# fabriziosestito/policy-server

Measured on AMD Instinct MI355X. Metric: admission requests evaluated/sec (node) at 64 policies; HBM GB/s vs peak, higher is better.
Workload: dtype u8; 1 GPU; C4: 1000000 synthetic Pod AdmissionReviews per GPU x 64 compiled policies (c4_64.yml: 22 psp-capabilities, 21 psp-apparmor, 21 safe-labels); config=c4_64, total_requests=1000000, policies=64, parallelism=dp1 (request shards)

## Files before the change

include/kwgpu.h:

```cpp
#ifndef KWGPU_H
#define KWGPU_H

#include <stddef.h>
#include <stdint.h>

#ifdef __cplusplus
extern "C" {
#endif

enum {
  KW_OK = 0,
  KW_E_INVALID_ID = 1,
  KW_E_INIT = 2,
  KW_E_NOT_FOUND = 3,
  KW_E_BOOTSTRAP = 4,
  KW_E_ENGINE = 5,
  KW_E_GROUP_REHYDRATE = 6,
  KW_E_ARG = 16,
  KW_E_PAYLOAD = 17,
  KW_E_DEVICE = 18,
  KW_E_NOSPACE = 19
};

enum { KW_MODE_PROTECT = 0, KW_MODE_MONITOR = 1 };
// ... 124 lines not shown
                       int origin, uint32_t *out);

int kw_debug_plan(const kw_env *env, kw_batch *b, const int32_t *policies, uint32_t npol, int origin, uint32_t *out,
                  int cap);

int kw_debug_copy_jobs(const kw_env *env, kw_batch *b, const int32_t *policies, uint32_t npol, int origin,
                       uint32_t *out, size_t cap, size_t *needed);

int kw_debug_tile_descs(const kw_env *env, kw_batch *b, const int32_t *policies, uint32_t npol, int origin,
                        uint32_t *out, size_t cap, size_t *needed);

uint64_t kw_debug_tile_cost(uint32_t feat, uint32_t need, uint32_t requests, uint32_t labels, uint32_t containers,
                            uint32_t capabilities);

int kw_debug_tile_slot(uint64_t ndesc, uint32_t grid, uint32_t workgroup, uint32_t tile, uint64_t *out);

int kw_debug_reorder(const kw_batch *b, uint64_t *perm, size_t cap, uint64_t *split, kw_batch **out);

int kw_validate_batch(const kw_env *env, kw_batch *b, const int32_t *policies, uint32_t npol,
                      int origin, void *stream);
int kw_validate_rows(const kw_env *env, kw_batch *b, const int32_t *row_policy, int origin,
                     void *stream);
int kw_batch_verdicts(kw_batch *b, uint32_t *host_out, size_t count);
int kw_validate_host(const kw_env *env, kw_batch *b, const int32_t *policies, uint32_t npol, int origin,
                     int device, uint32_t *out, size_t count, uint32_t chunk_rows);
typedef struct kw_packed {
  uint64_t rows;
  uint32_t npol;
  uint64_t *planes;
  uint32_t *exc_off;
// ... 83 lines not shown
```

policy-server_amd/csrc/capi.cpp:

```cpp
#include <hip/hip_runtime.h>

#include <algorithm>
#include <cstdio>
#include <cstdlib>
#include <cstring>
#include <memory>
#include <string>
#include <thread>
#include <vector>

#include "../../include/kwgpu.h"
#include "automaton.hpp"
#include "batch.hpp"
#include "devbatch.hpp"
#include "env.hpp"
#include "kernels.hpp"
#include "knobs.hpp"
#include "metrics.hpp"
#include "pass.hpp"
#include "plan.hpp"
#include "service.hpp"
#include "slotplan.hpp"
#include "upload.hpp"
#include "yaml.hpp"
// ... 633 lines not shown
}

uint64_t kw_debug_tile_cost(uint32_t feat, uint32_t need, uint32_t requests, uint32_t labels, uint32_t containers,
                            uint32_t capabilities) {
  return tile_cost(tile_cost_weights(feat, need), requests, labels, containers, capabilities);
}

int kw_debug_tile_slot(uint64_t ndesc, uint32_t grid, uint32_t workgroup, uint32_t tile, uint64_t* out) {
  if (!out || !grid || workgroup >= grid) return KW_E_ARG;
  const TileSlot s = tile_slot(ndesc, grid, workgroup);
  const uint64_t v[7] = {s.nx, s.xcd, s.slot, s.wpx, s.t_lo, s.t_hi, tile_at(s, tile)};
  std::copy(v, v + 7, out);
  return KW_OK;
}

int kw_debug_reorder(const kw_batch* kb, uint64_t* perm, size_t cap, uint64_t* split, kw_batch** out) {
  if (!kb || !split || !out || (!perm && kb->b.n) || cap < kb->b.n) return KW_E_ARG;
  std::vector<uint64_t> p;
  *split = split_rows(kb->b, &p);
  if (!*split) {
    p.resize(kb->b.n);
    for (uint64_t r = 0; r < kb->b.n; ++r) p[r] = r;
  }
  auto nb = std::make_unique<kw_batch>();
  RowOrder o;
  permute_batch(kb->b, p, &nb->b, true, &o);
  std::copy(p.begin(), p.end(), perm);
  *out = nb.release();
  return KW_OK;
}
// ... 136 lines not shown
```

policy-server_amd/csrc/devbatch.hpp:

```cpp
#pragma once
#include <hip/hip_runtime.h>

#include <atomic>
#include <cstdint>
#include <deque>
#include <memory>
#include <utility>
#include <vector>

#include "../../include/kwgpu.h"
#include "batch.hpp"
#include "env.hpp"
#include "kernels.hpp"
#include "pools.hpp"
#include "slotplan.hpp"

struct kw_env {
  kw::Env e;
  uint64_t uid = next_uid();
  static uint64_t next_uid() {
    static std::atomic<uint64_t> n{1};
    return n++;
  }
};
// ... 76 lines not shown
  uint32_t* verdicts = nullptr;
  size_t verdict_cap = 0;
  size_t last_verdicts = 0;
  uint32_t last_row_words = 0;
  std::vector<uint64_t> perm;
  std::vector<uint64_t> inv_perm;
  uint64_t split = 0;
  std::unique_ptr<Batch> dev_b;
  std::shared_ptr<PassPlan> plan_cache;
  uint64_t plan_env = 0, plan_knobs = 0;
  std::vector<int32_t> plan_pols;
  int plan_origin = -1;
  std::unique_ptr<RowOrder> order;
  uint32_t loaded = 0;
  uint32_t* sched = nullptr;
  hipEvent_t ev[3] = {nullptr, nullptr, nullptr};
  TileArgs* d_tiles = nullptr;
  size_t d_tiles_cap = 0;
  std::vector<TileArgs> h_tiles;
  uint8_t* d_slots = nullptr;
  size_t d_slots_cap = 0;
  std::vector<uint8_t> h_slots;
  uint32_t* rowcol = nullptr;
  size_t rowcol_cap = 0;
  std::vector<uint32_t> h_rowcol;
  TileDesc* desc = nullptr;
  size_t desc_cap = 0;
  uint32_t* overflow = nullptr;
  size_t overflow_cap = 0;
  std::vector<TileDesc> h_desc;
// ... 105 lines not shown
```

policy-server_amd/csrc/kernels.hip:

```cpp
#include <hip/hip_runtime.h>

#include <algorithm>
#include <array>
#include <cstddef>
#include <mutex>

#include "../../include/kwgpu.h"
#include "imgscan.hpp"
#include "kernels.hpp"


namespace kw {

typedef uint32_t u32x4 __attribute__((ext_vector_type(4)));

__device__ inline uint32_t lit_word(const uint32_t* base, uint32_t i, uint32_t sh, uint32_t len) {
  const uint32_t w = align_bytes(base[i + 1], base[i], sh);
  const uint32_t rem = len - 4u * i;
  return rem >= 4u ? w : (w & ((1u << (8u * rem)) - 1u));
}

template <bool BATCH, int N = 8>
__device__ inline uint32_t lit_lookup(const uint8_t* rec, const uint8_t* bytes, uint32_t b, uint32_t e) {
  const DevLit* L = (const DevLit*)rec;
// ... 433 lines not shown
  uint32_t* l_nx = (uint32_t*)(lds + t.o_nx);
  TileDesc* l_desc = (TileDesc*)(lds + t.o_desc);
  auto fetch_desc = [&](uint64_t i, uint32_t s) {
    if (tid < 32u)
      __builtin_amdgcn_global_load_lds((const __attribute__((address_space(1))) void*)((const uint32_t*)(desc + i) + tid),
                                       (__attribute__((address_space(3))) void*)(l_desc + s), 4, 0, 0);
  };
  auto sfield = [](const uint32_t& f) -> uint32_t { return __builtin_amdgcn_readfirstlane(f); };
  constexpr bool DYNB = !IMG;
  auto next_block = [&](uint32_t k) -> uint32_t {
    uint32_t v = 0;
    if (lane == 0u) v = atomicAdd(&l_nx[2u + k], 1u);
    return (kSlotThreads >> 6) + __builtin_amdgcn_readfirstlane(v);
  };
  const uint32_t wpx = (gridDim.x - xcd + nx - 1u) / nx;
  const uint64_t dbase = t_lo + 2ull * wpx;
  uint64_t tile = t_lo + blockIdx.x / nx, next = tile + wpx;
  constexpr bool desc_early = LDST;
  if (desc_early && tile < t_hi) fetch_desc(tile, 0);
  if (LDST) {
    for (uint32_t s = 0; s < t.nstage; ++s)
      glds_x4((const u32x4*)(a.blob + t.stage_blob[s]), (u32x4*)(lds + t.stage_lds[s]), t.stage_bytes[s] / 16u, tid);
    for (uint32_t c = 0; c < t.nchunk; ++c)
      glds_x4((const u32x4*)t.chunk[c].rec, (u32x4*)(lds + t.chunk[c].o_lds), ((const SlotHdr*)t.chunk[c].rec)->staged / 16u, tid);
  }
  __syncthreads();
  mark(7);
  const uint8_t* tb = LDST ? (const uint8_t*)lds : a.blob;
  Classifiers C;
#pragma unroll
  for (int c = 0; c < (int)NCOL; ++c) {
// ... 53 lines not shown
    const CopyJob q = tp->jobs[lane];
    jb_lo = (uint32_t)q.base;
    jb_hi = (uint32_t)(q.base >> 32);
    jb_code = q.code;
  }

  if (!desc_early) {
    if (tile < t_hi) fetch_desc(tile, 0);
    __syncthreads();
  }
  mark(4);
  for (uint32_t it = 0; tile < t_hi; ++it) {
    const uint64_t p0_t0 = timing ? clock64() : 0;
    const uint32_t cur = it & 1u;
    uint32_t nxt2 = 0;
    if (dyn && tid == 0) nxt2 = atomicAdd(cnt, 1u);
    if (next < t_hi) fetch_desc(next, cur ^ 1u);
    const TileDesc& d = l_desc[cur];
#define KW_DF(x) sfield(x)
    if (!KW_DF(d.fits)) {
      if (dyn && tid == 0) l_nx[cur] = nxt2;
      __syncthreads();
      tile = next;
      next = dyn ? dbase + l_nx[cur] : next + wpx;
      continue;
    }
    uint64_t p0_t1 = 0, p0_t2 = 0;
    if (timing) {
      p0_t1 = clock64();
      sg_add(SG_P0_TOP, p0_t1 - p0_t0);
    }

    {
      const uint32_t* dw = (const uint32_t*)&d;
      uint32_t code_v = jb_code;
      asm volatile("" : "+v"(code_v));
      const CopySpan sp = copy_span(code_v, dw[code_v & 31u], dw[(code_v >> 5) & 31u], d.r0hi);
      const uint64_t src = (((uint64_t)jb_hi << 32) | jb_lo) + sp.byte_off;
      const uint32_t s_lo = (uint32_t)src, s_hi = (uint32_t)(src >> 32);
// ... 563 lines not shown
          }
        }
      }
      if (timing) sg_add(SG_P3_BUSY, clock64() - p3_t0);
      if (ck + 1 < t.nchunk) {
        if (DYNB && tid == 0) l_nx[3] = 0;
        lds_barrier();
        mark(4);
      }
    }
    const uint64_t p3_end = timing ? clock64() : 0;
    lds_barrier();
    if (timing) sg_add(SG_P3_WAIT, clock64() - p3_end);
    mark(4);
    tile = next;
    next = dyn ? dbase + l_nx[cur] : next + wpx;
  }
  if (timing && tid == 0) {
    ph[6] = clock64() - t_begin;
    a.phase[(uint64_t)blockIdx.x * kPhaseWords + 8u + SG_END] = __builtin_amdgcn_s_memrealtime();
    for (int k = 0; k < 8; ++k) a.phase[(uint64_t)blockIdx.x * kPhaseWords + (uint32_t)k] = ph[k];
  }
  if (dyn && tid == 0) {
    uint32_t* done = a.sched + 256u + xcd * 32u;
    __threadfence();
    if (atomicAdd(done, 1u) == wpx - 1u) {
      atomicExch(cnt, 0u);
      atomicExch(done, 0u);
    }
  }
  (void)lane;
  (void)wave;
}

constexpr int kOverflowThreads = 256;

__device__ inline Classifiers blob_classifiers(const EvalArgs& a, const TileArgs& t) {
  Classifiers C;
  for (int c = 0; c < (int)NCOL; ++c) {
    C.lit[c] = t.lit_blob[c] ? a.blob + t.lit_blob[c] : nullptr;
// ... 322 lines not shown
  if (dev < 0 || dev >= kMaxDevices) return hipErrorInvalidDevice;
  std::call_once(g_attr_once[dev], [dev] {
    hipError_t e = hipSuccess;
    for (int k = 0; k < 70; ++k) {
      const uint32_t feat = k < 64 ? (uint32_t)(k >> 2) & kFeatAll : k < 68 ? (kFeatAll | kFeatNfa) : (kFeatLbl | kFeatCtr | kFeatRng);
      const hipError_t ek =
          hipFuncSetAttribute(tile_fn(k & 1, (k & 2) != 0, feat), hipFuncAttributeMaxDynamicSharedMemorySize, 160 * 1024);
      if (e == hipSuccess) e = ek;
    }
    g_attr_err[dev] = e;
  });
  return g_attr_err[dev];
}
}

hipError_t launch_evaluate_tiles(const EvalArgs& a, const TileArgs& t, const TileArgs* d_t, const TileDesc* d_desc,
                                 uint32_t grid, hipStream_t s) {
  if (a.nrows == 0 || t.nchunk == 0 || a.ndesc == 0) return hipSuccess;
  if (hipError_t e = ensure_attrs(); e != hipSuccess) return e;
  {
    thread_local int c_dev = -1, c_ncu = 0, c_occ = 0;
    thread_local uint64_t c_key = ~0ull;
    int dev = 0;
    const uint64_t key = ((uint64_t)t.lds_bytes << 8) | ((uint64_t)tile_feat(t) << 2) | (a.phase ? 2u : 0u) | (t.lds_tables ? 1u : 0u);
    if (hipGetDevice(&dev) == hipSuccess && (dev != c_dev || key != c_key)) {
      int ncu = 0, occ = 0;
      const void* fn = tile_fn(t.lds_tables != 0, a.phase != nullptr, tile_feat(t));
      if (hipDeviceGetAttribute(&ncu, hipDeviceAttributeMultiprocessorCount, dev) != hipSuccess ||
          hipOccupancyMaxActiveBlocksPerMultiprocessor(&occ, fn, kSlotThreads, t.lds_bytes) != hipSuccess)
        ncu = occ = 0;
      c_dev = dev;
      c_key = key;
      c_ncu = ncu;
      c_occ = occ;
    }
    c_occ = std::min<int>(c_occ, (int)lds_workgroups_per_cu(t.lds_bytes));
    if (c_occ > 0 && c_ncu > 0) grid = std::max<uint32_t>(1u, std::min<uint32_t>(grid, (uint32_t)(c_occ * c_ncu)));
    if (t.debug & 256u)
      fprintf(stderr, "[kw tile] launch grid=%u occupancy=%d wg/cu x %d CUs lds=%u\n", grid, c_occ, c_ncu, t.lds_bytes);
  }
  using TileFn = void (*)(EvalArgs, const TileArgs*, const TileDesc*);
  const TileFn fn = (TileFn)tile_fn(t.lds_tables != 0, a.phase != nullptr, tile_feat(t));
  hipLaunchKernelGGL(fn, dim3(grid), dim3(kSlotThreads), t.lds_bytes, s, a, d_t, d_desc);
  return hipGetLastError();
}

__global__ void __launch_bounds__(256) scatter_kernel(ScatterArgs a) {
  const uint64_t tid = (uint64_t)blockIdx.x * 256u + threadIdx.x, nt = (uint64_t)gridDim.x * 256u;
  for (uint32_t k = 0; k < a.nseg; ++k) {
    const ScatterSeg g = a.seg[k];
    uint8_t* d = a.dst + g.dst_off;
    const uint8_t* s = a.src + g.src_off;
    const uint64_t head = std::min<uint64_t>(g.bytes, (16u - ((uintptr_t)d & 15u)) & 15u);
    const uint64_t words = (g.bytes - head) / 16u, tail = g.bytes - head - words * 16u;
    if (tid < head) d[tid] = s[tid];
// ... 327 lines not shown
```

policy-server_amd/csrc/kernels.hpp:

```cpp
#pragma once
#include <hip/hip_runtime.h>

#include <cstdint>

#include "kwdev.hpp"
#include "packed.hpp"
#include "slots.hpp"
#include "summary.hpp"

namespace kw {

enum Str : uint32_t { S_NS = 0, S_IMG, S_AA, S_CAPADD, S_CAPDROP, S_LK, S_LV, NSTR };

struct WideRec {
  uint32_t row_lo, row_hi, policy, value;
};

struct EvalArgs {
  const uint8_t* blob;
  uint64_t nrows;
  uint64_t ndesc;
  uint32_t npol;
  int32_t origin;
  const uint8_t* req_flags;
  const uint32_t* ctr_off;
  const uint32_t* lbl_off;
  const uint8_t* ctr_flags;
  const uint32_t* capadd_off;
  const uint32_t* capdrop_off;
  uint32_t* out;
  uint32_t* sched;
  uint16_t *g_ns, *g_aa, *g_img, *g_capadd, *g_capdrop, *g_lk, *g_lv;
  const uint16_t *nfa_lv, *nfa_img;
  uint32_t* wide_count;
  WideRec* wide_rec;
  uint32_t wide_cap;
  uint64_t* wide_groups;
  uint32_t nwide;
  const uint32_t* rowcol;
  uint64_t* phase;
};
enum Seg : uint32_t {
  SG_P1_LABEL = 0, SG_P1_CAPSTR, SG_P1_CTR, SG_P1_IMAGE, SG_P1_REQ, SG_P2_CTR, SG_P2_LABEL, SG_P2_REQ,
  SG_P1_BUSY, SG_P1_WAIT, SG_P2_BUSY, SG_P2_WAIT, SG_P0_WAIT, SG_P3_BUSY, SG_P3_WAIT,
  SG_START,
  SG_P0_TOP, SG_P0_REQ, SG_P0_STR,
// ... 110 lines not shown
struct TileSlot {
  uint32_t nx, xcd, slot, wpx;
  uint64_t t_lo, t_hi;
};
KW_HD inline TileSlot tile_slot(uint64_t ndesc, uint32_t grid, uint32_t b) {
  TileSlot s;
  s.nx = grid < 8u ? grid : 8u;
  s.xcd = b % s.nx;
  s.slot = b / s.nx;
  s.wpx = (grid - s.xcd + s.nx - 1u) / s.nx;
  s.t_lo = ndesc * s.xcd / s.nx;
  s.t_hi = ndesc * (s.xcd + 1u) / s.nx;
  return s;
}
KW_HD inline uint64_t tile_at(const TileSlot& s, uint32_t k) { return s.t_lo + s.slot + (uint64_t)k * s.wpx; }

struct TileCostW {
  uint32_t fixed, req, lbl, ctr, cap;
};
KW_HD constexpr uint32_t tile_blocks(uint32_t items) { return (items + 63u) / 64u; }
KW_HD constexpr uint64_t tile_cost(const TileCostW& w, uint32_t nreq, uint32_t nlbl, uint32_t nctr, uint32_t ncap) {
  return (uint64_t)w.fixed + (uint64_t)w.req * tile_blocks(nreq) + (uint64_t)w.lbl * tile_blocks(nlbl) +
         (uint64_t)w.ctr * tile_blocks(nctr) + (uint64_t)w.cap * tile_blocks(ncap);
}
KW_HD constexpr TileCostW tile_cost_weights(uint32_t feat, uint32_t need) {
  TileCostW w{47000u, 8450u, 0u, 0u, 0u};
  if ((feat & kFeatLbl) && (need & (1u << S_LK))) w.lbl = 9960u;
  if (feat & kFeatCtr) w.ctr = 10600u;
  if ((feat & kFeatCtr) && (need & (1u << S_CAPADD))) w.cap = 2750u;
  if ((feat & kFeatImg) && (need & (1u << S_IMG))) w.ctr = 35600u;
  return w;
}

void build_copy_jobs(TileArgs* T, const void* const cols[6]);

hipError_t launch_evaluate_tiles(const EvalArgs& a, const TileArgs& t, const TileArgs* d_t, const TileDesc* d_desc,
                                 uint32_t grid, hipStream_t s);
struct WideGroupArgs {
  uint32_t prog_off, prog_len;
  uint32_t col;
  uint32_t nmem, midx_off;
  uint32_t okw, rejb;
  uint32_t cause_off, cause_words;
  uint32_t errw;
  uint32_t kind;
  uint32_t mutw;
};

constexpr uint32_t kSplitMember = 0x80000000u;
// ... 97 lines not shown
```

policy-server_amd/csrc/knobs.hpp:

```cpp
#pragma once
#include <climits>
#include <cstddef>
#include <cstdint>

namespace kw {

enum Knob : int {
  KW_STREAM_POOL, KW_HOST_THREADS, KW_L2_PREFETCH, KW_KV_GLOBAL, KW_NO_MPACK,
  KW_BULK_DEBUG, KW_BULK_SAMPLE, KW_BULK_PACK, KW_BULK_CHUNK, KW_BULK_RAMP, KW_BULK_DIRECT, KW_BULK_DEPTH,
  KW_SCHED, KW_SPLIT, KW_GROUP_FORM, KW_POISON_VERDICTS, KW_FLATTEN_THREADS,
  KW_SLOT_ROWS, KW_HEAVY_ROWS, KW_HEAVY_CTR, KW_GLOBAL_TABLES, KW_TILE_SPLIT, KW_ROUND_SPLIT,
  KW_TILE_QUANTILE, KW_TILE_DEBUG, KW_TILE_CUT,
  KW_NKNOBS
};

enum class KnobKind : uint8_t {
  On,
  Off,
  Present,
  Int,
  Double,
  Str
};

struct KnobRow {
// ... 21 lines not shown

constexpr KnobRow kKnobs[KW_NKNOBS] = {
    knob_flag("KW_STREAM_POOL", KnobKind::On, kLatched, kNoPlan, "reuse streams and events per device"),
    knob_int("KW_HOST_THREADS", kLatched, kNoPlan, 0, 1, INT_MAX, kClamp, "host worker threads (unset: the hardware's, at most 16)"),
    knob_flag("KW_L2_PREFETCH", KnobKind::Off, kLatched, kPlans, "run the next-tile L2 prefetch (kernels built with KW_PREFETCH)"),
    knob_flag("KW_KV_GLOBAL", KnobKind::Off, kLatched, kPlans, "label-value DFAs read from global memory, not staged"),
    knob_flag("KW_NO_MPACK", KnobKind::Present, kLatched, kPlans, "slot plans without mandatory-field batching"),
    knob_flag("KW_BULK_DEBUG", KnobKind::Off, kLatched, kNoPlan, "print host stage times of planning and the bulk path"),
    knob_flag("KW_BULK_SAMPLE", KnobKind::On, kLatched, kNoPlan, "bulk path: tile capacities from ~2048 sampled tiles"),
    knob_flag("KW_BULK_PACK", KnobKind::On, kLatched, kNoPlan, "bulk path: packed chunks through their own ring"),
    knob_int("KW_BULK_CHUNK", kLatched, kNoPlan, 262144, 1, INT_MAX, kClamp, "bulk path: rows per chunk"),
    knob_flag("KW_BULK_RAMP", KnobKind::On, kLatched, kNoPlan, "bulk path: small first and last chunks"),
    knob_flag("KW_BULK_DIRECT", KnobKind::On, kLatched, kNoPlan, "bulk path: read back straight into pinned output"),
    knob_int("KW_BULK_DEPTH", kLatched, kNoPlan, -1, 0, INT_MAX, kClamp, "bulk path: chunks in flight (0: unbounded; unset: 2 or 3)"),
    knob_flag("KW_SCHED", KnobKind::Str, kLive, kPlans, "static / dynamic: force one tile schedule"),
    knob_int("KW_SPLIT", kLive, kPlans, -1, INT_MIN, INT_MAX, kClamp, "0: never split light / heavy rows, 1: whenever both exist"),
    knob_flag("KW_GROUP_FORM", KnobKind::Str, kLive, kPlans, "script: compile every group expression as a script"),
    knob_flag("KW_POISON_VERDICTS", KnobKind::Off, kLive, kPlans, "fill the verdict words with a sentinel before a pass"),
    knob_int("KW_FLATTEN_THREADS", kLive, kNoPlan, 0, 1, INT_MAX, kClamp, "JSON flatten threads (unset: the hardware's, at most 16)"),
    knob_int("KW_SLOT_ROWS", kLive, kPlans, 0, 8, 255, kElseUnset, "force the tile height"),
    knob_int("KW_HEAVY_ROWS", kLive, kPlans, 0, 8, 255, kElseUnset, "force the heavy region's tile height"),
    knob_int("KW_HEAVY_CTR", kLive, kPlans, 5, 1, INT_MAX, kElseUnset, "containers above which a request is heavy"),
    knob_flag("KW_GLOBAL_TABLES", KnobKind::Off, kLive, kPlans, "classifier tables read from global memory"),
    knob_real("KW_TILE_SPLIT", kPlans, 0.02, "share of tiles a capacity choice may split"),
    knob_real("KW_ROUND_SPLIT", kPlans, 0.02, "share of a taller tile's tiles that may need a second P1 round"),
    knob_real("KW_TILE_QUANTILE", kPlans, 0.0, "force the capacity quantile (unset: chosen per batch)"),
    knob_int("KW_TILE_DEBUG", kLive, kPlans, 0, INT_MIN, INT_MAX, kClamp, "kernel phase ablation bits; 256: print the plan"),
    knob_flag("KW_TILE_CUT", KnobKind::On, kLive, kPlans, "end each tile at the row of least estimated cost per row (0: fixed height)"),
};

constexpr bool knob_name_is(const char* a, const char* b) {
  while (*a && *a == *b) ++a, ++b;
  return *a == *b;
}
#define KW_KNOB_ROW(K) static_assert(knob_name_is(kKnobs[K].name, #K), "kKnobs is not in Knob order")
KW_KNOB_ROW(KW_STREAM_POOL); KW_KNOB_ROW(KW_HOST_THREADS); KW_KNOB_ROW(KW_L2_PREFETCH); KW_KNOB_ROW(KW_KV_GLOBAL);
KW_KNOB_ROW(KW_NO_MPACK); KW_KNOB_ROW(KW_BULK_DEBUG); KW_KNOB_ROW(KW_BULK_SAMPLE); KW_KNOB_ROW(KW_BULK_PACK);
KW_KNOB_ROW(KW_BULK_CHUNK); KW_KNOB_ROW(KW_BULK_RAMP); KW_KNOB_ROW(KW_BULK_DIRECT); KW_KNOB_ROW(KW_BULK_DEPTH);
KW_KNOB_ROW(KW_SCHED); KW_KNOB_ROW(KW_SPLIT); KW_KNOB_ROW(KW_GROUP_FORM); KW_KNOB_ROW(KW_POISON_VERDICTS);
KW_KNOB_ROW(KW_FLATTEN_THREADS); KW_KNOB_ROW(KW_SLOT_ROWS); KW_KNOB_ROW(KW_HEAVY_ROWS); KW_KNOB_ROW(KW_HEAVY_CTR);
KW_KNOB_ROW(KW_GLOBAL_TABLES); KW_KNOB_ROW(KW_TILE_SPLIT); KW_KNOB_ROW(KW_ROUND_SPLIT); KW_KNOB_ROW(KW_TILE_QUANTILE);
KW_KNOB_ROW(KW_TILE_DEBUG); KW_KNOB_ROW(KW_TILE_CUT);
#undef KW_KNOB_ROW

uint64_t kw_knob_hash();

namespace knob_detail {

const char* env(const KnobRow& r);
bool parse_bool(const KnobRow& r);
int parse_int(const KnobRow& r);
double parse_double(const KnobRow& r);

template <Knob K>
// ... 60 lines not shown
```

policy-server_amd/csrc/pass.cpp:

```cpp
#include "pass.hpp"

#include <atomic>
#include <chrono>
#include <cstdio>
#include <cstring>
#include <memory>

#include "knobs.hpp"
#include "plan.hpp"

namespace kw {

int upload_env(kw_env* env, int device) {
  if (device < 0) return KW_OK;
  HIPCHK(hipSetDevice(device));
  HIPCHK(hipMalloc(&env->e.d_blob, env->e.blob.size()));
  HIPCHK(hipMemcpy(env->e.d_blob, env->e.blob.data(), env->e.blob.size(), hipMemcpyHostToDevice));
  env->e.device = device;
  return KW_OK;
}

int build_descs(const Batch& B, const TileArgs& T, uint64_t lo, uint64_t hi, uint64_t t0, uint64_t t1, uint64_t range,
                uint32_t grid, std::vector<TileDesc>* desc, std::vector<uint32_t>* ovf) {
  auto make = [&](uint64_t r0, uint64_t r1, TileDesc* dp) {
// ... 262 lines not shown
    D.desc_valid = false;
    D.ndesc = 0;
    D.reg_ndesc[0] = D.reg_ndesc[1] = 0;
    D.n_overflow = 0;
  }
  A.ndesc = D.ndesc;
  if (Knobs::on<KW_POISON_VERDICTS>())
    HIPCHK(hipMemsetAsync(D.verdicts, 0xA5, D.last_verdicts * sizeof(uint32_t), s));
  if (!D.sched) {
    void* p = nullptr;
    HIPCHK(dev_pool().alloc(D.device, 512 * sizeof(uint32_t), &p));
    D.sched = (uint32_t*)p;
    HIPCHK(hipMemsetAsync(D.sched, 0, 512 * sizeof(uint32_t), s));
  }
  A.sched = D.sched;
  if (plan.nwide) {
    if (int rc = ensure(&D.wide_groups, &D.wide_groups_cap, (size_t)(B.n * plan.nwide))) return rc;
    A.wide_groups = D.wide_groups;
  }
  if (!D.wide_count) {
    void* p = nullptr;
    HIPCHK(dev_pool().alloc(D.device, sizeof(uint32_t), &p));
    D.wide_count = (uint32_t*)p;
  }
  D.wide_valid = D.n_overflow != 0;
  if (D.wide_valid) HIPCHK(hipMemsetAsync(D.wide_count, 0, sizeof(uint32_t), s));
  A.wide_count = D.wide_count;
  if (D.n_overflow) {
    if (int rc = ensure_overflow_classes(B, &D, plan.geom, &A)) return rc;
    const size_t cap = (size_t)D.n_overflow * plan.wide_cap_per_row;
// ... 1 lines not shown
    A.wide_rec = D.wide_rec;
    A.wide_cap = (uint32_t)std::min<size_t>(cap, 0xffffffffu);
  }
  if (plan.geom.feat & kFeatNfa) {
    if (int rc = ensure_nfa(kb, plan, &A)) return rc;
  }
  D.last_nwide = plan.nwide;
  D.last_wide_policy = plan.wide_policy;
  D.last_rows_mode = plan.rows_mode;
  D.last_row_words = plan.args.npol;
  D.last_wide_cap = A.wide_cap;
  *out_args = A;
  return KW_OK;
}

static void print_phase_report(size_t launch, uint32_t grid, const std::vector<uint64_t>& ph) {
  double sum[kPhaseWords] = {0};
  for (uint32_t g = 0; g < grid; ++g)
    for (uint32_t k = 0; k < kPhaseWords; ++k) sum[k] += (double)ph[(size_t)g * kPhaseWords + k];
  const double tiles = std::max(1.0, sum[5]);
  fprintf(stderr,
          "[kw phase] launch %zu grid %u tiles %.0f: cycles/tile P0 %.0f P1 %.0f D %.0f P2 %.0f P3+next %.0f "
          "(sum %.0f); per workgroup: %.0f cycles, %.2f tiles, table staging %.0f\n",
          launch, grid, tiles, sum[0] / tiles, sum[1] / tiles, sum[2] / tiles, sum[3] / tiles, sum[4] / tiles,
          (sum[0] + sum[1] + sum[2] + sum[3] + sum[4]) / tiles, sum[6] / grid, tiles / grid, sum[7] / grid);
  const double wt = tiles * (double)(kSlotThreads / 64u);
  const double* g = sum + 8;
  fprintf(stderr,
          "[kw seg] per wave-tile: P0 wait %.0f | P1 busy %.0f wait %.0f (label %.0f capstr %.0f ctr %.0f image %.0f req %.0f) "
          "| P2 busy %.0f wait %.0f (ctr %.0f label %.0f req %.0f) | P3 busy %.0f wait %.0f | P0 issue: top to fits %.0f "
          "job spans %.0f job loop %.0f\n",
// ... 21 lines not shown
    for (uint32_t q = x; q < grid; q += nx) {
      const uint64_t* w = &ph[(size_t)q * kPhaseWords + 8];
      if (!w[SG_START] || !w[SG_END]) continue;
      ++n;
      first = std::min(first, w[SG_START]);
      e_lo = std::min(e_lo, w[SG_END]);
      e_hi = std::max(e_hi, w[SG_END]);
      ends += w[SG_END];
    }
    const double idle = (double)n * (double)e_hi - (double)ends, span = (double)n * (double)(e_hi - first);
    idle_all += idle;
    span_all += span;
    stamped += (uint32_t)n;
    fprintf(stderr, " %.1f / %.1f %%", (double)(e_hi - e_lo) / 100.0, span > 0 ? 100.0 * idle / span : 0.0);
  }
  fprintf(stderr, " (all: %.1f %% idle; %u of %u workgroups stamped)\n", span_all > 0 ? 100.0 * idle_all / span_all : 0.0,
          stamped, grid);
}

static int run_pass(kw_batch* kb, PassPlan& plan, bool timed, hipStream_t s) {
  DeviceBatch& D = *kb->dev;
  EvalArgs A;
  if (int rc = prepare_pass(kb, plan, s, &A)) return rc;
  const bool phases = (plan.geom.debug & 512u) != 0;
  void* d_phase = nullptr;
  uint32_t gmax = 0;
  for (const PassPlan::Region& rg : plan.regions) gmax = std::max(gmax, rg.grid);
  const size_t phase_bytes = (size_t)gmax * kPhaseWords * sizeof(uint64_t);
  if (phases) {
    HIPCHK(hipMalloc(&d_phase, phase_bytes));
    A.phase = (uint64_t*)d_phase;
  }
  if (timed) HIPCHK(hipEventRecord(D.ev[0], s));
  if (plan.geom.feat & kFeatNfa) HIPCHK(launch_nfa_classify(A, D.d_tiles, plan.nfa, plan.nfa_threads, s));
  const size_t nl = plan.launches.size();
  for (size_t l = 0; l < plan.tiles.size(); ++l) {
    const size_t k = l / nl;
    if (phases) HIPCHK(hipMemsetAsync(d_phase, 0, phase_bytes, s));
    const uint32_t grid = plan.regions[k].grid;
    EvalArgs Ak = A;
    Ak.ndesc = D.reg_ndesc[k];
    if (!plan.regions[k].dyn) Ak.sched = nullptr;
    HIPCHK(launch_evaluate_tiles(Ak, plan.tiles[l], D.d_tiles + l, D.desc + D.reg_desc[k], grid, s));
    if (phases) {
      std::vector<uint64_t> ph((size_t)grid * kPhaseWords);
      HIPCHK(hipMemcpyAsync(ph.data(), d_phase, ph.size() * sizeof(uint64_t), hipMemcpyDeviceToHost, s));
      HIPCHK(hipStreamSynchronize(s));
      print_phase_report(l, grid, ph);
    }
    if (D.n_overflow && k + 1 == plan.regions.size()) HIPCHK(launch_overflow(A, D.d_tiles + l, D.overflow, D.n_overflow, s));
  }
  if (timed) HIPCHK(hipEventRecord(D.ev[2], s));
  if (phases) HIPCHK(hipFree(d_phase));
  return KW_OK;
}

int run_validate(const kw_env* env, kw_batch* kb, PassPlan& plan, int origin, bool timed, hipStream_t s) {
  DeviceBatch& D = *kb->dev;
  const PassPlan::Wide& W = plan.wide;
  D.last_big_stride = 0;
  D.last_big_ref.clear();
  if (W.groups.empty()) return run_pass(kb, plan, timed, s);
  const uint64_t n = kb->b.n;
// ... 233 lines not shown
```

policy-server_amd/csrc/plan.cpp:

```cpp
#define KW_PLANNING_TU
#include "plan.hpp"

#include <algorithm>
#include <chrono>
#include <cstdio>
#include <cstring>
#include <map>

#include "knobs.hpp"
#include "slots.hpp"

namespace kw {

bool sched_dynamic(uint64_t ntiles, uint32_t grid, bool lds_tables) {
  const char* e = PlanKnobs::str<KW_SCHED>();
  if (!strcmp(e, "static")) return false;
  if (!strcmp(e, "dynamic")) return true;
  return ntiles > (lds_tables ? 16ull : 4ull) * std::max<uint32_t>(grid, 1);
}

namespace {

uint32_t heavy_rows() { return (uint32_t)PlanKnobs::num<KW_HEAVY_ROWS>(); }

uint32_t slot_rows_forced() { return (uint32_t)PlanKnobs::num<KW_SLOT_ROWS>(); }

bool l2_prefetch() { return KW_PREFETCH && PlanKnobs::on<KW_L2_PREFETCH>(); }

}

void str_range(const Batch& B, int m, uint64_t r0, uint64_t r1, uint64_t* g0, uint64_t* g1) {
  switch (m) {
    case S_NS: *g0 = r0; *g1 = r1; break;
// ... 720 lines not shown
```

policy-server_amd/csrc/plan.hpp:

```cpp
#pragma once
#include <cstdint>
#include <vector>

#include "devbatch.hpp"

namespace kw {

void str_range(const Batch& B, int m, uint64_t r0, uint64_t r1, uint64_t* g0, uint64_t* g1);

bool sched_dynamic(uint64_t ntiles, uint32_t grid, bool lds_tables);

void plan_wide_groups(const Env& E, const std::vector<int32_t>& list, const std::vector<uint32_t>* rows_code,
                      int origin, PassPlan* plan);

int plan_pass(const kw_env* env, kw_batch* kb, const int32_t* pols, uint32_t npol, const int32_t* row_policy,
              int origin, bool timing, PassPlan* plan);

}
```

policy-server_amd/kwgpu/__init__.py:

```python
import ctypes as C
import json

from . import _native as N
from ._native import KwSoa, KwTiming

PROTECT, MONITOR = N.KW_MODE_PROTECT, N.KW_MODE_MONITOR
VALIDATE, AUDIT = N.KW_ORIGIN_VALIDATE, N.KW_ORIGIN_AUDIT


class RequestOrigin:
    Validate = N.KW_ORIGIN_VALIDATE
    Audit = N.KW_ORIGIN_AUDIT


class PolicyMode:
    Protect = N.KW_MODE_PROTECT
    Monitor = N.KW_MODE_MONITOR


class EvaluationError(Exception):

    code = None

    def __init__(self, message, code=None):
# ... 531 lines not shown
        return out[:need.value]

    def debug_tile_descs(self, env, policies, origin=VALIDATE):
        import numpy as np
        arr = env._array(policies)
        need = C.c_size_t()
        rc = self._L.kw_debug_tile_descs(env._h, self._h, arr, len(policies), origin, None, 0, C.byref(need))
        if rc != N.KW_E_NOSPACE:
            raise_for(rc, "kw_debug_tile_descs failed")
        out = np.zeros(max(need.value, 1), dtype=np.uint32)
        rc = self._L.kw_debug_tile_descs(env._h, self._h, arr, len(policies), origin,
                                         out.ctypes.data_as(C.POINTER(C.c_uint32)), out.size, C.byref(need))
        raise_for(rc, "kw_debug_tile_descs failed")
        return out[:need.value]

    def debug_reorder(self):
        import numpy as np
        perm = np.zeros(max(self.n, 1), dtype=np.uint64)
        split, h = C.c_uint64(), C.c_void_p()
        rc = self._L.kw_debug_reorder(self._h, perm.ctypes.data_as(C.POINTER(C.c_uint64)), len(perm), C.byref(split),
                                      C.byref(h))
        raise_for(rc, "kw_debug_reorder failed")
        return Batch(h.value), perm[:self.n], split.value

    def wide_arg(self, row, policy):
        v = C.c_uint64()
        rc = self._L.kw_batch_wide_arg(self._h, row, policy, C.byref(v))
        return v.value if rc == N.KW_OK else None

    def group_causes(self, row, policy, verdict):
# ... 204 lines not shown
```

policy-server_amd/kwgpu/_native.py:

```python
import ctypes as C
import os

PKG_DIR = os.path.dirname(os.path.dirname(os.path.abspath(__file__)))
LIB_PATH = os.environ.get("KWGPU_LIB") or os.path.join(PKG_DIR, "libkwgpu.so")
SYNTH_PATH = os.path.join(PKG_DIR, "libkwsynth.so")

KW_OK = 0
KW_E_INVALID_ID = 1
KW_E_INIT = 2
KW_E_NOT_FOUND = 3
KW_E_BOOTSTRAP = 4
KW_E_ENGINE = 5
KW_E_GROUP_REHYDRATE = 6
KW_E_ARG = 16
KW_E_PAYLOAD = 17
KW_E_DEVICE = 18
KW_E_NOSPACE = 19

KW_MODE_PROTECT = 0
KW_MODE_MONITOR = 1
KW_ORIGIN_VALIDATE = 0
KW_ORIGIN_AUDIT = 1
KW_DOC_ADMISSION_REVIEW = 0
KW_DOC_RAW_REVIEW = 1
# ... 57 lines not shown
                ("dict", C.POINTER(C.c_uint32)), ("exc_count", C.c_size_t)]


class KwSummary(C.Structure):
    _fields_ = [("rows", C.c_uint64), ("npol", C.c_uint32), ("col", C.POINTER(C.c_uint64)),
                ("planes", C.POINTER(C.c_uint64))]


EXPORTS = [
    "kw_env_build", "kw_env_build_yaml", "kw_yaml_to_json", "kw_env_serialize", "kw_env_deserialize", "kw_env_destroy", "kw_env_lookup",
    "kw_env_policy_count", "kw_env_policy_id", "kw_env_is_group", "kw_env_get_policy_mode",
    "kw_env_get_policy_allowed_to_mutate",
    "kw_env_should_always_accept_requests_made_inside_of_namespace",
    "kw_env_policy_initialization_error", "kw_env_validate_settings", "kw_pattern_match", "kw_pattern_match_many", "kw_env_pattern_count",
    "kw_env_pattern", "kw_env_classify", "kw_batch_wide_arg", "kw_batch_group_causes", "kw_debug_plan", "kw_debug_copy_jobs", "kw_debug_reorder",
    "kw_debug_tile_descs", "kw_debug_tile_cost", "kw_debug_tile_slot",
    "kw_batch_from_json", "kw_batch_from_soa", "kw_batch_view", "kw_batch_to_device", "kw_batch_to_device_async",
    "kw_stream_create", "kw_stream_destroy", "kw_validate_host", "kw_validate_host_packed", "kw_packed_word",
    "kw_packed_unpack", "kw_debug_pack_words", "kw_batch_summary", "kw_validate_host_summary", "kw_batch_verdict_rows",
    "kw_batch_last_pass",
    "kw_debug_summarize_words", "kw_batch_pin_host", "kw_host_alloc", "kw_host_free",
    "kw_batch_destroy", "kw_debug_host_walk", "kw_validate_batch", "kw_validate_rows", "kw_batch_verdicts",
    "kw_validate_timed", "kw_format_response", "kw_format_response_doc", "kw_env_group_members", "kw_evaluate",
    "kw_service_constraints", "kw_metrics_create", "kw_metrics_destroy", "kw_metrics_record", "kw_metrics_render",
    "kw_metrics_reset", "kw_version",
]

_lib = None
_synth = None


# ... 26 lines not shown
        "kw_env_should_always_accept_requests_made_inside_of_namespace": (ip, [vp, cp, sz]),
        "kw_env_policy_initialization_error": (ip, [vp, i32, cp, sz]),
        "kw_env_validate_settings": (ip, [vp, i32, cp, sz]),
        "kw_pattern_match": (ip, [ip, cp, cp, sz]),
        "kw_pattern_match_many": (ip, [ip, cp, C.POINTER(cp), C.POINTER(sz), sz, C.POINTER(C.c_int32)]),
        "kw_env_pattern_count": (ip, [vp, ip]),
        "kw_env_pattern": (ip, [vp, ip, ip, C.POINTER(ip), cp, sz]),
        "kw_env_classify": (ip, [vp, ip, cp, sz, cp, sz, C.POINTER(u32), ip]),
        "kw_batch_wide_arg": (ip, [vp, u64, i32, C.POINTER(u64)]),
        "kw_batch_group_causes": (ip, [vp, u64, i32, C.c_uint32, C.POINTER(u64), C.c_size_t, C.POINTER(C.c_size_t)]),
        "kw_debug_plan": (ip, [vp, vp, C.POINTER(i32), u32, ip, C.POINTER(u32), ip]),
        "kw_debug_copy_jobs": (ip, [vp, vp, C.POINTER(i32), u32, ip, C.POINTER(u32), sz, C.POINTER(sz)]),
        "kw_debug_tile_descs": (ip, [vp, vp, C.POINTER(i32), u32, ip, C.POINTER(u32), sz, C.POINTER(sz)]),
        "kw_debug_tile_cost": (u64, [u32, u32, u32, u32, u32, u32]),
        "kw_debug_tile_slot": (ip, [u64, u32, u32, u32, C.POINTER(u64)]),
        "kw_debug_reorder": (ip, [vp, C.POINTER(u64), sz, C.POINTER(u64), C.POINTER(vp)]),
        "kw_batch_from_json": (ip, [C.POINTER(cp), C.POINTER(sz), sz, ip, C.POINTER(vp), C.POINTER(C.c_int64), cp, sz]),
        "kw_batch_from_soa": (ip, [C.POINTER(KwSoa), C.POINTER(vp)]),
        "kw_batch_view": (ip, [vp, C.POINTER(KwSoa)]),
        "kw_batch_to_device": (ip, [vp, ip]),
        "kw_batch_to_device_async": (ip, [vp, ip, vp]),
        "kw_stream_create": (ip, [ip, C.POINTER(vp)]),
        "kw_stream_destroy": (None, [vp]),
        "kw_batch_destroy": (None, [vp]),
        "kw_validate_batch": (ip, [vp, vp, C.POINTER(i32), u32, ip, vp]),
        "kw_validate_rows": (ip, [vp, vp, C.POINTER(i32), ip, vp]),
        "kw_batch_verdicts": (ip, [vp, C.POINTER(u32), sz]),
        "kw_validate_host": (ip, [vp, vp, C.POINTER(i32), u32, ip, ip, C.POINTER(u32), sz, u32]),
        "kw_validate_host_packed": (ip, [vp, vp, C.POINTER(i32), u32, ip, ip, C.POINTER(KwPacked), u32]),
        "kw_packed_word": (ip, [C.POINTER(KwPacked), u64, u32, C.POINTER(u32)]),
# ... 54 lines not shown
```

Before: 4.300 billion requests/s.

## Add dynamic tail to static tile schedule with per-launch round selection

```diff
diff --git a/include/kwgpu.h b/include/kwgpu.h
--- a/include/kwgpu.h
+++ b/include/kwgpu.h
@@ -162,6 +162,12 @@
                             uint32_t capabilities);
 
 int kw_debug_tile_slot(uint64_t ndesc, uint32_t grid, uint32_t workgroup, uint32_t tile, uint64_t *out);
+
+int kw_debug_sched_tail(uint64_t ndesc, uint32_t grid, uint32_t workgroup, uint32_t rounds, uint64_t *out);
+
+int kw_debug_sched_rounds(uint64_t ndesc, uint32_t grid, int dynamic, int *rounds);
+
+int kw_debug_last_launches(const kw_batch *b, int64_t *out, size_t cap, size_t *needed);
 
 int kw_debug_reorder(const kw_batch *b, uint64_t *perm, size_t cap, uint64_t *split, kw_batch **out);
 
diff --git a/policy-server_amd/csrc/capi.cpp b/policy-server_amd/csrc/capi.cpp
--- a/policy-server_amd/csrc/capi.cpp
+++ b/policy-server_amd/csrc/capi.cpp
@@ -671,6 +671,32 @@
   return KW_OK;
 }
 
+int kw_debug_sched_tail(uint64_t ndesc, uint32_t grid, uint32_t workgroup, uint32_t rounds, uint64_t* out) {
+  if (!out || !grid || workgroup >= grid) return KW_E_ARG;
+  const TileSlot s = tile_slot(ndesc, grid, workgroup);
+  const uint64_t tail = tile_tail_lo(s, rounds);
+  const uint64_t first = s.t_lo + s.slot;
+  const uint64_t v[7] = {s.t_lo, s.slot, s.wpx, tail > first ? (tail - first + s.wpx - 1) / s.wpx : 0, tail, s.t_hi,
+                         tile_whole_rounds(ndesc, grid)};
+  std::copy(v, v + 7, out);
+  return KW_OK;
+}
+
+int kw_debug_sched_rounds(uint64_t ndesc, uint32_t grid, int dynamic, int* rounds) {
+  if (!rounds || !grid) return KW_E_ARG;
+  *rounds = sched_static_rounds(ndesc, grid, dynamic != 0);
+  return KW_OK;
+}
+
+int kw_debug_last_launches(const kw_batch* kb, int64_t* out, size_t cap, size_t* needed) {
+  if (!kb || !kb->dev || !needed || (!out && cap)) return KW_E_ARG;
+  const std::vector<int64_t>& v = kb->dev->last_launches;
+  *needed = v.size();
+  if (cap < v.size()) return KW_E_NOSPACE;
+  std::copy(v.begin(), v.end(), out);
+  return KW_OK;
+}
+
 int kw_debug_reorder(const kw_batch* kb, uint64_t* perm, size_t cap, uint64_t* split, kw_batch** out) {
   if (!kb || !split || !out || (!perm && kb->b.n) || cap < kb->b.n) return KW_E_ARG;
   std::vector<uint64_t> p;
diff --git a/policy-server_amd/csrc/devbatch.hpp b/policy-server_amd/csrc/devbatch.hpp
--- a/policy-server_amd/csrc/devbatch.hpp
+++ b/policy-server_amd/csrc/devbatch.hpp
@@ -114,6 +114,7 @@
   std::unique_ptr<RowOrder> order;
   uint32_t loaded = 0;
   uint32_t* sched = nullptr;
+  std::vector<int64_t> last_launches;
   hipEvent_t ev[3] = {nullptr, nullptr, nullptr};
   TileArgs* d_tiles = nullptr;
   size_t d_tiles_cap = 0;
diff --git a/policy-server_amd/csrc/kernels.hip b/policy-server_amd/csrc/kernels.hip
--- a/policy-server_amd/csrc/kernels.hip
+++ b/policy-server_amd/csrc/kernels.hip
@@ -471,7 +471,7 @@
     return (kSlotThreads >> 6) + __builtin_amdgcn_readfirstlane(v);
   };
   const uint32_t wpx = (gridDim.x - xcd + nx - 1u) / nx;
-  const uint64_t dbase = t_lo + 2ull * wpx;
+  const uint64_t dbase = dyn ? t_lo + (uint64_t)a.sched_static * wpx : 0;
   uint64_t tile = t_lo + blockIdx.x / nx, next = tile + wpx;
   constexpr bool desc_early = LDST;
   if (desc_early && tile < t_hi) fetch_desc(tile, 0);
@@ -555,7 +555,15 @@
     const uint64_t p0_t0 = timing ? clock64() : 0;
     const uint32_t cur = it & 1u;
     uint32_t nxt2 = 0;
-    if (dyn && tid == 0) nxt2 = atomicAdd(cnt, 1u);
+    if (dyn && tid == 0) {
+      if (next + wpx >= dbase) {
+        auto* c = (__attribute__((address_space(1))) uint32_t*)cnt;
+        asm volatile("" : "+v"(c));
+        nxt2 = __hip_atomic_fetch_add(c, 1u, __ATOMIC_RELAXED, __HIP_MEMORY_SCOPE_AGENT);
+      } else {
+        nxt2 = (uint32_t)(next + wpx - dbase);
+      }
+    }
     if (next < t_hi) fetch_desc(next, cur ^ 1u);
     const TileDesc& d = l_desc[cur];
 #define KW_DF(x) sfield(x)
@@ -563,7 +571,7 @@
       if (dyn && tid == 0) l_nx[cur] = nxt2;
       __syncthreads();
       tile = next;
-      next = dyn ? dbase + l_nx[cur] : next + wpx;
+      next = dyn ? dbase + (uint64_t)(int64_t)(int32_t)l_nx[cur] : next + wpx;
       continue;
     }
     uint64_t p0_t1 = 0, p0_t2 = 0;
@@ -1157,7 +1165,7 @@
     if (timing) sg_add(SG_P3_WAIT, clock64() - p3_end);
     mark(4);
     tile = next;
-    next = dyn ? dbase + l_nx[cur] : next + wpx;
+    next = dyn ? dbase + (uint64_t)(int64_t)(int32_t)l_nx[cur] : next + wpx;
   }
   if (timing && tid == 0) {
     ph[6] = clock64() - t_begin;
@@ -1166,7 +1174,7 @@
   }
   if (dyn && tid == 0) {
     uint32_t* done = a.sched + 256u + xcd * 32u;
-    __threadfence();
+    __builtin_amdgcn_fence(__ATOMIC_SEQ_CST, "wavefront");
     if (atomicAdd(done, 1u) == wpx - 1u) {
       atomicExch(cnt, 0u);
       atomicExch(done, 0u);
@@ -1519,31 +1527,35 @@
 }
 }
 
+uint32_t tile_launch_grid(const TileArgs& t, bool timing, uint32_t grid, bool print) {
+  if (ensure_attrs() != hipSuccess) return grid;
+  thread_local int c_dev = -1, c_ncu = 0, c_occ = 0;
+  thread_local uint64_t c_key = ~0ull;
+  int dev = 0;
+  const uint64_t key = ((uint64_t)t.lds_bytes << 8) | ((uint64_t)tile_feat(t) << 2) | (timing ? 2u : 0u) | (t.lds_tables ? 1u : 0u);
+  if (hipGetDevice(&dev) == hipSuccess && (dev != c_dev || key != c_key)) {
+    int ncu = 0, occ = 0;
+    const void* fn = tile_fn(t.lds_tables != 0, timing, tile_feat(t));
+    if (hipDeviceGetAttribute(&ncu, hipDeviceAttributeMultiprocessorCount, dev) != hipSuccess ||
+        hipOccupancyMaxActiveBlocksPerMultiprocessor(&occ, fn, kSlotThreads, t.lds_bytes) != hipSuccess)
+      ncu = occ = 0;
+    c_dev = dev;
+    c_key = key;
+    c_ncu = ncu;
+    c_occ = occ;
+  }
+  c_occ = std::min<int>(c_occ, (int)lds_workgroups_per_cu(t.lds_bytes));
+  if (c_occ > 0 && c_ncu > 0) grid = std::max<uint32_t>(1u, std::min<uint32_t>(grid, (uint32_t)(c_occ * c_ncu)));
+  if (print && (t.debug & 256u))
+    fprintf(stderr, "[kw tile] launch grid=%u occupancy=%d wg/cu x %d CUs lds=%u\n", grid, c_occ, c_ncu, t.lds_bytes);
+  return grid;
+}
+
 hipError_t launch_evaluate_tiles(const EvalArgs& a, const TileArgs& t, const TileArgs* d_t, const TileDesc* d_desc,
                                  uint32_t grid, hipStream_t s) {
   if (a.nrows == 0 || t.nchunk == 0 || a.ndesc == 0) return hipSuccess;
   if (hipError_t e = ensure_attrs(); e != hipSuccess) return e;
-  {
-    thread_local int c_dev = -1, c_ncu = 0, c_occ = 0;
-    thread_local uint64_t c_key = ~0ull;
-    int dev = 0;
-    const uint64_t key = ((uint64_t)t.lds_bytes << 8) | ((uint64_t)tile_feat(t) << 2) | (a.phase ? 2u : 0u) | (t.lds_tables ? 1u : 0u);
-    if (hipGetDevice(&dev) == hipSuccess && (dev != c_dev || key != c_key)) {
-      int ncu = 0, occ = 0;
-      const void* fn = tile_fn(t.lds_tables != 0, a.phase != nullptr, tile_feat(t));
-      if (hipDeviceGetAttribute(&ncu, hipDeviceAttributeMultiprocessorCount, dev) != hipSuccess ||
-          hipOccupancyMaxActiveBlocksPerMultiprocessor(&occ, fn, kSlotThreads, t.lds_bytes) != hipSuccess)
-        ncu = occ = 0;
-      c_dev = dev;
-      c_key = key;
-      c_ncu = ncu;
-      c_occ = occ;
-    }
-    c_occ = std::min<int>(c_occ, (int)lds_workgroups_per_cu(t.lds_bytes));
-    if (c_occ > 0 && c_ncu > 0) grid = std::max<uint32_t>(1u, std::min<uint32_t>(grid, (uint32_t)(c_occ * c_ncu)));
-    if (t.debug & 256u)
-      fprintf(stderr, "[kw tile] launch grid=%u occupancy=%d wg/cu x %d CUs lds=%u\n", grid, c_occ, c_ncu, t.lds_bytes);
-  }
+  grid = tile_launch_grid(t, a.phase != nullptr, grid, true);
   using TileFn = void (*)(EvalArgs, const TileArgs*, const TileDesc*);
   const TileFn fn = (TileFn)tile_fn(t.lds_tables != 0, a.phase != nullptr, tile_feat(t));
   hipLaunchKernelGGL(fn, dim3(grid), dim3(kSlotThreads), t.lds_bytes, s, a, d_t, d_desc);
diff --git a/policy-server_amd/csrc/kernels.hpp b/policy-server_amd/csrc/kernels.hpp
--- a/policy-server_amd/csrc/kernels.hpp
+++ b/policy-server_amd/csrc/kernels.hpp
@@ -30,6 +30,7 @@
   const uint32_t* capdrop_off;
   uint32_t* out;
   uint32_t* sched;
+  uint32_t sched_static;
   uint16_t *g_ns, *g_aa, *g_img, *g_capadd, *g_capdrop, *g_lk, *g_lv;
   const uint16_t *nfa_lv, *nfa_img;
   uint32_t* wide_count;
@@ -170,6 +171,20 @@
   return s;
 }
 KW_HD inline uint64_t tile_at(const TileSlot& s, uint32_t k) { return s.t_lo + s.slot + (uint64_t)k * s.wpx; }
+KW_HD inline uint64_t tile_tail_lo(const TileSlot& s, uint32_t S) {
+  const uint64_t lo = s.t_lo + (uint64_t)S * s.wpx;
+  return lo < s.t_hi ? lo : s.t_hi;
+}
+KW_HD inline uint64_t tile_whole_rounds(uint64_t ndesc, uint32_t grid) {
+  uint64_t q = ~0ull;
+  const uint32_t nx = grid < 8u ? grid : 8u;
+  for (uint32_t x = 0; x < nx; ++x) {
+    const TileSlot s = tile_slot(ndesc, grid, x);
+    const uint64_t r = (s.t_hi - s.t_lo) / s.wpx;
+    q = r < q ? r : q;
+  }
+  return nx ? q : 0;
+}
 
 struct TileCostW {
   uint32_t fixed, req, lbl, ctr, cap;
@@ -189,6 +204,8 @@
 }
 
 void build_copy_jobs(TileArgs* T, const void* const cols[6]);
+
+uint32_t tile_launch_grid(const TileArgs& t, bool timing, uint32_t grid, bool print = false);
 
 hipError_t launch_evaluate_tiles(const EvalArgs& a, const TileArgs& t, const TileArgs* d_t, const TileDesc* d_desc,
                                  uint32_t grid, hipStream_t s);
diff --git a/policy-server_amd/csrc/knobs.hpp b/policy-server_amd/csrc/knobs.hpp
--- a/policy-server_amd/csrc/knobs.hpp
+++ b/policy-server_amd/csrc/knobs.hpp
@@ -8,7 +8,7 @@
 enum Knob : int {
   KW_STREAM_POOL, KW_HOST_THREADS, KW_L2_PREFETCH, KW_KV_GLOBAL, KW_NO_MPACK,
   KW_BULK_DEBUG, KW_BULK_SAMPLE, KW_BULK_PACK, KW_BULK_CHUNK, KW_BULK_RAMP, KW_BULK_DIRECT, KW_BULK_DEPTH,
-  KW_SCHED, KW_SPLIT, KW_GROUP_FORM, KW_POISON_VERDICTS, KW_FLATTEN_THREADS,
+  KW_SCHED, KW_SCHED_TAIL, KW_SPLIT, KW_GROUP_FORM, KW_POISON_VERDICTS, KW_FLATTEN_THREADS,
   KW_SLOT_ROWS, KW_HEAVY_ROWS, KW_HEAVY_CTR, KW_GLOBAL_TABLES, KW_TILE_SPLIT, KW_ROUND_SPLIT,
   KW_TILE_QUANTILE, KW_TILE_DEBUG, KW_TILE_CUT,
   KW_NKNOBS
@@ -60,6 +60,7 @@
     knob_flag("KW_BULK_DIRECT", KnobKind::On, kLatched, kNoPlan, "bulk path: read back straight into pinned output"),
     knob_int("KW_BULK_DEPTH", kLatched, kNoPlan, -1, 0, INT_MAX, kClamp, "bulk path: chunks in flight (0: unbounded; unset: 2 or 3)"),
     knob_flag("KW_SCHED", KnobKind::Str, kLive, kPlans, "static / dynamic: force one tile schedule"),
+    knob_int("KW_SCHED_TAIL", kLive, kPlans, -1, 0, INT_MAX, kElseUnset, "rounds a strided launch draws from the counters at its end (0: none; unset: chosen per launch)"),
     knob_int("KW_SPLIT", kLive, kPlans, -1, INT_MIN, INT_MAX, kClamp, "0: never split light / heavy rows, 1: whenever both exist"),
     knob_flag("KW_GROUP_FORM", KnobKind::Str, kLive, kPlans, "script: compile every group expression as a script"),
     knob_flag("KW_POISON_VERDICTS", KnobKind::Off, kLive, kPlans, "fill the verdict words with a sentinel before a pass"),
@@ -83,7 +84,7 @@
 KW_KNOB_ROW(KW_STREAM_POOL); KW_KNOB_ROW(KW_HOST_THREADS); KW_KNOB_ROW(KW_L2_PREFETCH); KW_KNOB_ROW(KW_KV_GLOBAL);
 KW_KNOB_ROW(KW_NO_MPACK); KW_KNOB_ROW(KW_BULK_DEBUG); KW_KNOB_ROW(KW_BULK_SAMPLE); KW_KNOB_ROW(KW_BULK_PACK);
 KW_KNOB_ROW(KW_BULK_CHUNK); KW_KNOB_ROW(KW_BULK_RAMP); KW_KNOB_ROW(KW_BULK_DIRECT); KW_KNOB_ROW(KW_BULK_DEPTH);
-KW_KNOB_ROW(KW_SCHED); KW_KNOB_ROW(KW_SPLIT); KW_KNOB_ROW(KW_GROUP_FORM); KW_KNOB_ROW(KW_POISON_VERDICTS);
+KW_KNOB_ROW(KW_SCHED); KW_KNOB_ROW(KW_SCHED_TAIL); KW_KNOB_ROW(KW_SPLIT); KW_KNOB_ROW(KW_GROUP_FORM); KW_KNOB_ROW(KW_POISON_VERDICTS);
 KW_KNOB_ROW(KW_FLATTEN_THREADS); KW_KNOB_ROW(KW_SLOT_ROWS); KW_KNOB_ROW(KW_HEAVY_ROWS); KW_KNOB_ROW(KW_HEAVY_CTR);
 KW_KNOB_ROW(KW_GLOBAL_TABLES); KW_KNOB_ROW(KW_TILE_SPLIT); KW_KNOB_ROW(KW_ROUND_SPLIT); KW_KNOB_ROW(KW_TILE_QUANTILE);
 KW_KNOB_ROW(KW_TILE_DEBUG); KW_KNOB_ROW(KW_TILE_CUT);
diff --git a/policy-server_amd/csrc/pass.cpp b/policy-server_amd/csrc/pass.cpp
--- a/policy-server_amd/csrc/pass.cpp
+++ b/policy-server_amd/csrc/pass.cpp
@@ -300,6 +300,7 @@
     HIPCHK(hipMemsetAsync(D.sched, 0, 512 * sizeof(uint32_t), s));
   }
   A.sched = D.sched;
+  A.sched_static = 2;
   if (plan.nwide) {
     if (int rc = ensure(&D.wide_groups, &D.wide_groups_cap, (size_t)(B.n * plan.nwide))) return rc;
     A.wide_groups = D.wide_groups;
@@ -331,7 +332,7 @@
   return KW_OK;
 }
 
-static void print_phase_report(size_t launch, uint32_t grid, const std::vector<uint64_t>& ph) {
+static void print_phase_report(size_t launch, uint32_t grid, const std::vector<uint64_t>& ph, uint64_t ndesc, int S) {
   double sum[kPhaseWords] = {0};
   for (uint32_t g = 0; g < grid; ++g)
     for (uint32_t k = 0; k < kPhaseWords; ++k) sum[k] += (double)ph[(size_t)g * kPhaseWords + k];
@@ -383,8 +384,24 @@
     stamped += (uint32_t)n;
     fprintf(stderr, " %.1f / %.1f %%", (double)(e_hi - e_lo) / 100.0, span > 0 ? 100.0 * idle / span : 0.0);
   }
-  fprintf(stderr, " (all: %.1f %% idle; %u of %u workgroups stamped)\n", span_all > 0 ? 100.0 * idle_all / span_all : 0.0,
+  fprintf(stderr, " (all: %.1f %% idle; %u of %u workgroups stamped)", span_all > 0 ? 100.0 * idle_all / span_all : 0.0,
           stamped, grid);
+  uint64_t t_min = ~0ull, t_max = 0;
+  for (uint32_t q = 0; q < grid; ++q) {
+    const uint64_t n = ph[(size_t)q * kPhaseWords + 5];
+    t_min = std::min(t_min, n);
+    t_max = std::max(t_max, n);
+  }
+  fprintf(stderr, "; tiles per workgroup min %llu mean %.2f max %llu", (unsigned long long)(grid ? t_min : 0), tiles / std::max(grid, 1u),
+          (unsigned long long)t_max);
+  if (S >= 0) {
+    fprintf(stderr, "; S %d, tail tiles per XCD:", S);
+    for (uint32_t x = 0; x < nx; ++x) {
+      const TileSlot ts = tile_slot(ndesc, grid, x);
+      fprintf(stderr, " %llu", (unsigned long long)(ts.t_hi - tile_tail_lo(ts, (uint32_t)S)));
+    }
+  }
+  fprintf(stderr, "\n");
 }
 
 static int run_pass(kw_batch* kb, PassPlan& plan, bool timed, hipStream_t s) {
@@ -403,19 +420,23 @@
   if (timed) HIPCHK(hipEventRecord(D.ev[0], s));
   if (plan.geom.feat & kFeatNfa) HIPCHK(launch_nfa_classify(A, D.d_tiles, plan.nfa, plan.nfa_threads, s));
   const size_t nl = plan.launches.size();
+  D.last_launches.clear();
   for (size_t l = 0; l < plan.tiles.size(); ++l) {
     const size_t k = l / nl;
     if (phases) HIPCHK(hipMemsetAsync(d_phase, 0, phase_bytes, s));
-    const uint32_t grid = plan.regions[k].grid;
+    const uint32_t grid = tile_launch_grid(plan.tiles[l], phases, plan.regions[k].grid);
     EvalArgs Ak = A;
     Ak.ndesc = D.reg_ndesc[k];
-    if (!plan.regions[k].dyn) Ak.sched = nullptr;
+    const int S = sched_static_rounds(Ak.ndesc, grid, plan.regions[k].dyn);
+    if (S < 0) Ak.sched = nullptr;
+    else Ak.sched_static = (uint32_t)S;
+    for (int64_t v : {(int64_t)grid, (int64_t)Ak.ndesc, (int64_t)S}) D.last_launches.push_back(v);
     HIPCHK(launch_evaluate_tiles(Ak, plan.tiles[l], D.d_tiles + l, D.desc + D.reg_desc[k], grid, s));
     if (phases) {
       std::vector<uint64_t> ph((size_t)grid * kPhaseWords);
       HIPCHK(hipMemcpyAsync(ph.data(), d_phase, ph.size() * sizeof(uint64_t), hipMemcpyDeviceToHost, s));
       HIPCHK(hipStreamSynchronize(s));
-      print_phase_report(l, grid, ph);
+      print_phase_report(l, grid, ph, Ak.ndesc, S);
     }
     if (D.n_overflow && k + 1 == plan.regions.size()) HIPCHK(launch_overflow(A, D.d_tiles + l, D.overflow, D.n_overflow, s));
   }
diff --git a/policy-server_amd/csrc/plan.cpp b/policy-server_amd/csrc/plan.cpp
--- a/policy-server_amd/csrc/plan.cpp
+++ b/policy-server_amd/csrc/plan.cpp
@@ -17,6 +17,18 @@
   if (!strcmp(e, "static")) return false;
   if (!strcmp(e, "dynamic")) return true;
   return ntiles > (lds_tables ? 16ull : 4ull) * std::max<uint32_t>(grid, 1);
+}
+
+constexpr uint32_t kSchedTail = 2, kSchedTailMinRounds = 7;
+int sched_static_rounds(uint64_t ndesc, uint32_t grid, bool dyn) {
+  const int forced = PlanKnobs::num<KW_SCHED_TAIL>();
+  const int today = dyn ? 2 : -1;
+  const char* e = PlanKnobs::str<KW_SCHED>();
+  if (!strcmp(e, "static") || !strcmp(e, "dynamic") || forced == 0 || !grid) return today;
+  const uint64_t q = tile_whole_rounds(ndesc, grid);
+  if (forced > 0) return q >= (uint64_t)forced + 2 ? (int)std::min<uint64_t>(q - (uint64_t)forced, INT_MAX) : today;
+  if (dyn || q < kSchedTailMinRounds) return today;
+  return (int)std::min<uint64_t>(q - kSchedTail, INT_MAX);
 }
 
 namespace {
diff --git a/policy-server_amd/csrc/plan.hpp b/policy-server_amd/csrc/plan.hpp
--- a/policy-server_amd/csrc/plan.hpp
+++ b/policy-server_amd/csrc/plan.hpp
@@ -9,6 +9,7 @@
 void str_range(const Batch& B, int m, uint64_t r0, uint64_t r1, uint64_t* g0, uint64_t* g1);
 
 bool sched_dynamic(uint64_t ntiles, uint32_t grid, bool lds_tables);
+int sched_static_rounds(uint64_t ndesc, uint32_t grid, bool dyn);
 
 void plan_wide_groups(const Env& E, const std::vector<int32_t>& list, const std::vector<uint32_t>* rows_code,
                       int origin, PassPlan* plan);
diff --git a/policy-server_amd/kwgpu/__init__.py b/policy-server_amd/kwgpu/__init__.py
--- a/policy-server_amd/kwgpu/__init__.py
+++ b/policy-server_amd/kwgpu/__init__.py
@@ -569,6 +569,16 @@
         raise_for(rc, "kw_debug_tile_descs failed")
         return out[:need.value]
 
+    def debug_last_launches(self):
+        need = C.c_size_t()
+        rc = self._L.kw_debug_last_launches(self._h, None, 0, C.byref(need))
+        if rc != N.KW_E_NOSPACE:
+            raise_for(rc, "kw_debug_last_launches failed")
+            return []
+        out = (C.c_int64 * need.value)()
+        raise_for(self._L.kw_debug_last_launches(self._h, out, need.value, C.byref(need)), "kw_debug_last_launches failed")
+        return [tuple(out[i:i + 3]) for i in range(0, need.value, 3)]
+
     def debug_reorder(self):
         import numpy as np
         perm = np.zeros(max(self.n, 1), dtype=np.uint64)
diff --git a/policy-server_amd/kwgpu/_native.py b/policy-server_amd/kwgpu/_native.py
--- a/policy-server_amd/kwgpu/_native.py
+++ b/policy-server_amd/kwgpu/_native.py
@@ -95,7 +95,7 @@
     "kw_env_should_always_accept_requests_made_inside_of_namespace",
     "kw_env_policy_initialization_error", "kw_env_validate_settings", "kw_pattern_match", "kw_pattern_match_many", "kw_env_pattern_count",
     "kw_env_pattern", "kw_env_classify", "kw_batch_wide_arg", "kw_batch_group_causes", "kw_debug_plan", "kw_debug_copy_jobs", "kw_debug_reorder",
-    "kw_debug_tile_descs", "kw_debug_tile_cost", "kw_debug_tile_slot",
+    "kw_debug_tile_descs", "kw_debug_tile_cost", "kw_debug_tile_slot", "kw_debug_sched_tail", "kw_debug_sched_rounds", "kw_debug_last_launches",
     "kw_batch_from_json", "kw_batch_from_soa", "kw_batch_view", "kw_batch_to_device", "kw_batch_to_device_async",
     "kw_stream_create", "kw_stream_destroy", "kw_validate_host", "kw_validate_host_packed", "kw_packed_word",
     "kw_packed_unpack", "kw_debug_pack_words", "kw_batch_summary", "kw_validate_host_summary", "kw_batch_verdict_rows",
@@ -152,6 +152,9 @@
         "kw_debug_tile_descs": (ip, [vp, vp, C.POINTER(i32), u32, ip, C.POINTER(u32), sz, C.POINTER(sz)]),
         "kw_debug_tile_cost": (u64, [u32, u32, u32, u32, u32, u32]),
         "kw_debug_tile_slot": (ip, [u64, u32, u32, u32, C.POINTER(u64)]),
+        "kw_debug_sched_tail": (ip, [u64, u32, u32, u32, C.POINTER(u64)]),
+        "kw_debug_sched_rounds": (ip, [u64, u32, ip, C.POINTER(ip)]),
+        "kw_debug_last_launches": (ip, [vp, C.POINTER(C.c_int64), sz, C.POINTER(sz)]),
         "kw_debug_reorder": (ip, [vp, C.POINTER(u64), sz, C.POINTER(u64), C.POINTER(vp)]),
         "kw_batch_from_json": (ip, [C.POINTER(cp), C.POINTER(sz), sz, ip, C.POINTER(vp), C.POINTER(C.c_int64), cp, sz]),
         "kw_batch_from_soa": (ip, [C.POINTER(KwSoa), C.POINTER(vp)]),
```

After: 4.589 billion requests/s (median of 6 runs). 1.07x the previous value.
